# ETM-Code/eirgrid

Hardware: AMD Instinct MI355X
Metric: 26-year episodes/sec (higher is better)
Workload: dtype f64

## Files before the change

eirgrid_amd/csrc/eg_api.cpp:

```cpp
#include <algorithm>
#include <cstdlib>
#include <cstring>

#include "eg_device_tables.h"
#include "eg_host.h"
#include "eg_policy_internal.h"

namespace eg {
namespace {
thread_local std::string g_error;
}
void set_error(const std::string& s) { g_error = s; }
}

using namespace eg;

void eg_host_tables::index() {
  auto F = [&](const char* n, const std::vector<double>& v) { f64[n] = {v.data(), (int64_t)v.size()}; };
  auto I = [&](const char* n, const std::vector<int32_t>& v) { i32[n] = {v.data(), (int64_t)v.size()}; };
  F("usage", H.usage); F("population", H.population); F("pre_co2", H.pre_co2); F("pre_tg", H.pre_tg); F("pre_ig", H.pre_ig);
  F("pre_sg", H.pre_sg); F("pre_optot", H.pre_optot); F("te", H.te); F("coastf", H.coastf); F("dr", H.dr); F("m03", H.m03);
  F("t12", H.t12); F("cc", H.cc); F("out_mw", H.out_mw); F("co2_t", H.co2_t); F("offv", H.offv); F("offc", H.offc);
  F("inflation", H.inflation); F("carbon_price", H.carbon_price);
  f64["size_factor"] = {&H.size_factor, 1};
// ... 4 lines not shown
namespace {
struct Options {
  bool helper_off = false, helper_all = false;
  bool heavy_slots_auto = true; uint32_t heavy_slots_wanted = 4096;
  uint32_t heavy_slots_max = 0;
  bool side_stream_plain = false;
  bool replay_hoist = false;
  int coop_force = 0;
  bool solo_on = true;
  uint32_t solo_tiles = 1u;
};
Options read_options() {
  Options o;
  if (const char* hv = std::getenv("EIRGRID_HELPER_WAVES")) { o.helper_off = std::string(hv) == "0"; o.helper_all = std::string(hv) == "all"; }
  if (const char* hs = std::getenv("EIRGRID_HEAVY_SLOTS")) { o.heavy_slots_wanted = (uint32_t)std::strtoul(hs, nullptr, 10); o.heavy_slots_auto = false; }
  o.heavy_slots_max = uint32_t((size_t(64) << 30) / (size_t(kRadiusClasses) * 2624 * sizeof(double)));
  if (const char* hg = std::getenv("EIRGRID_HEAVY_POOL_GB"))
    o.heavy_slots_max = uint32_t(std::min(double((1u << 20) - 1u), std::max(0.0, std::atof(hg)) * double(size_t(1) << 30) / double(size_t(kRadiusClasses) * 2624 * sizeof(double))));
  if (o.heavy_slots_max > (1u << 20) - 1u) o.heavy_slots_max = (1u << 20) - 1u;
  if (o.heavy_slots_wanted > o.heavy_slots_max) o.heavy_slots_wanted = o.heavy_slots_max;
  if (const char* sp = std::getenv("EIRGRID_SIDE_STREAM")) o.side_stream_plain = std::string(sp) == "plain";
  if (const char* rh = std::getenv("EIRGRID_REPLAY_HOIST")) o.replay_hoist = rh[0] == '1';
  if (const char* cf = std::getenv("EIRGRID_COOP_FORCE")) o.coop_force = std::atoi(cf);
  if (const char* so = std::getenv("EIRGRID_REPLAY_SOLO")) o.solo_on = so[0] != '0';
  if (const char* st = std::getenv("EIRGRID_SOLO_TILES")) o.solo_tiles = st[0] != '0' ? 1u : 0u;
  return o;
}

int collect_timing(eg_ctx* c, int count = -1) {
  if (count < 0 || count > c->ring_pending) count = c->ring_pending;
  for (; count > 0; --count) {
    const int i = (c->ring_head - c->ring_pending + 2 * eg_ctx::kTimingRing) % eg_ctx::kTimingRing;
    const bool heavy = c->ev_used[i] & 1, lean = c->ev_used[i] & 2;
    float best = 0.f, sum = 0.f;
    for (int a = 0; a < 2; ++a)
      for (int b = 0; b < 2; ++b) {
        if (!(a ? lean : heavy) || !(b ? lean : heavy)) continue;
        EG_HIP(hipEventSynchronize(c->ev[i][2 * b + 1]));
        float ms = 0.f;
        EG_HIP(hipEventElapsedTime(&ms, c->ev[i][2 * a], c->ev[i][2 * b + 1]));
        if (a == b) sum += ms;
        if (ms > best) best = ms;
      }
    c->total_ms += double(best); c->grids_ms += double(sum); c->n_launches += 1; c->ring_pending -= 1;
  }
  return EG_OK;
}
}
static bool env_starts(const char* name, char ch) { const char* e = std::getenv(name); return e && e[0] == ch; }
bool eg::stats_replicas_off() { static const bool off = env_starts("EIRGRID_STATS_REPLICAS", '0'); return off; }
bool eg::fetch_full() { static const bool full = env_starts("EIRGRID_FETCH_FULL", '1'); return full; }

int eg::ensure_outputs(eg_ctx* c, uint32_t n) {
  const size_t bytes = size_t(n) * rec::stride + size_t(n) * sizeof(double);
  if (bytes <= c->d_out.count) return EG_OK;
  c->out = DevOut{};
  EG_HIP(c->d_out.reserve(bytes));
  c->out.base = c->d_out;
  c->out.score_list = reinterpret_cast<double*>(c->out.base + size_t(n) * rec::stride);
  EG_HIP(hipMemset(c->out.base, 0, bytes));
  return EG_OK;
}

int eg::ring_take(eg_ctx* c, RolloutPlan& plan, int& slot) {
  if (c->ring_pending == eg_ctx::kTimingRing) EG_TRY(collect_timing(c, 1));
  slot = c->ring_head;
  for (int k = 0; k < 4; ++k) plan.ev[k] = c->ev[slot][k];
  return EG_OK;
}
void eg::ring_commit(eg_ctx* c, int slot, int ev_used) {
  c->ev_used[slot] = uint8_t(ev_used);
  c->ring_head = (c->ring_head + 1) % eg_ctx::kTimingRing; c->ring_pending += 1;
}
int eg::arm_solo(eg_ctx* c, RolloutPlan& plan, uint32_t n) {
  if (!c->solo_on) return EG_OK;
  bool fresh = false;
  EG_HIP(c->d_solo.reserve(n, &fresh));
  if (fresh) EG_HIP(hipMemsetAsync(c->d_solo, 0, sizeof(unsigned long long) * n, nullptr));
  plan.solo_seq = ++c->solo_seq; plan.d_solo = c->d_solo;
  return EG_OK;
}

int eg::prepare_heavy(eg_ctx* c, uint32_t n_heavy, bool known_short) {
  constexpr size_t kSlotBytes = size_t(kRadiusClasses) * 2624 * sizeof(double), kTileBytes = size_t(kMaxVariants) * 64 * sizeof(double);
  if (known_short && !c->dev.heavy) n_heavy = 0;
  uint32_t want = c->heavy_slots_wanted;
  if (c->heavy_slots_auto && want > 0) {
    while (want < n_heavy && want < c->heavy_slots_max) want = want * 2u < c->heavy_slots_max ? want * 2u : c->heavy_slots_max;
  }
  if (want > 0 && n_heavy > 0 && (!c->dev.heavy || want > c->dev.heavy_slots)) {
    if (c->dev.heavy) {
      EG_HIP(hipDeviceSynchronize());
      c->d_heavy.release();
      c->dev.heavy = nullptr; c->dev.heavy_slots = 0; c->dev.heavy_tiles = nullptr;
    }
    if (!c->dev.heavy_claim) {
      if (!c->d_heavy_claim.try_reserve(16)) { c->heavy_slots_wanted = 0; want = 0; }
      else { EG_HIP(hipMemset(c->d_heavy_claim, 0xFF, 64)); c->dev.heavy_claim = c->d_heavy_claim; }
    }
    while (want > 0 && !c->d_heavy.try_reserve((kSlotBytes + kTileBytes) * want)) {
      want = want > 4096u ? want / 2u : 0u;
      c->heavy_slots_auto = false; c->heavy_slots_wanted = want;
    }
    if (want > 0) {
      c->dev.heavy = c->d_heavy; c->dev.heavy_slots = want;
      c->dev.heavy_tiles = reinterpret_cast<double*>(c->d_heavy + kSlotBytes * want);
    }
  }
  c->launch_epoch = (c->launch_epoch + 1u) & 0xFFFu;
  if (c->launch_epoch == 0xFFFu) c->launch_epoch = 0u;
  c->dev.heavy_epoch = c->launch_epoch;
  return EG_OK;
}

namespace {
int launch_batch(eg_ctx* c, uint64_t seed, uint64_t first_index, uint32_t n, const uint8_t* host_mask, uint32_t period, long long* d_stats) {
  if (n == 0) return EG_OK;
  RolloutPlan plan{};
  plan.helper_waves = n <= c->helper_max_episodes;
  plan.n_lean = n;
  const uint8_t* d_mask = nullptr;
  if (host_mask) {
    EG_HIP(c->d_mask.reserve(n));
    EG_HIP(c->d_index.reserve(n));
    std::vector<uint32_t> idx(n);
    uint32_t nh = 0;
    for (uint32_t i = 0; i < n; ++i) if (host_mask[i]) idx[nh++] = i;
    uint32_t k = nh;
    for (uint32_t i = 0; i < n; ++i) if (!host_mask[i]) idx[k++] = i;
    EG_HIP(hipMemcpy(c->d_mask, host_mask, n, hipMemcpyHostToDevice));
    EG_HIP(hipMemcpy(c->d_index, idx.data(), sizeof(uint32_t) * n, hipMemcpyHostToDevice));
    d_mask = c->d_mask;
    plan.n_heavy = nh; plan.n_lean = n - nh; plan.mode = 1u; plan.d_index = c->d_index;
  } else if (period == 1u) {
    plan.n_heavy = n; plan.n_lean = 0;
  } else if (period > 1u) {
    plan.off = uint32_t((uint64_t(period) - first_index % period) % period);
    plan.n_heavy = plan.off < n ? (n - plan.off + period - 1u) / period : 0u;
    plan.n_lean = n - plan.n_heavy; plan.mode = 2u; plan.period = period;
  }
  int slot = 0;
  EG_TRY(ring_take(c, plan, slot));
  const bool split = plan.n_heavy > 0 && plan.n_lean > 0;
  plan.stream_heavy = split ? c->stream_heavy : nullptr;
  plan.stream_lean = nullptr;
  bool list_long = c->long_list_hint;
  if (!c->list_exact && c->h_list_len) list_long = *(volatile uint32_t*)c->h_list_len > uint32_t(kShortReplayMax);
  plan.skip_long = c->list_exact && !list_long;
  EG_TRY(prepare_heavy(c, plan.n_heavy, plan.skip_long));
  if (d_stats != nullptr) {
    const bool off = stats_replicas_off();
    if (!off && n >= 4096u) {
      bool fresh = false;
      EG_HIP(c->d_stats_rep.reserve(size_t(kStatsReplicas) * EG_STATS_LEN, &fresh));
      if (fresh) EG_HIP(hipMemsetAsync(c->d_stats_rep, 0, sizeof(long long) * size_t(kStatsReplicas) * EG_STATS_LEN, nullptr));
    }
    plan.d_stats_rep = (off || n < 4096u) ? nullptr : c->d_stats_rep;
    if (plan.d_stats_rep != nullptr && c->stats_rep_dirty) {
      if (c->stream_heavy) EG_HIP(hipStreamSynchronize(c->stream_heavy));
      EG_HIP(hipMemsetAsync(c->d_stats_rep, 0, sizeof(long long) * size_t(kStatsReplicas) * EG_STATS_LEN, nullptr));
      c->stats_rep_dirty = false;
    }
  }
  if (plan.n_heavy > 0 && !plan.helper_waves && !plan.skip_long && !c->hoist_on)
    EG_TRY(arm_solo(c, plan, plan.n_heavy));
  if (c->hoist_on && plan.n_heavy > 0) {
    plan.hoist_seq = ++c->hoist_seq; plan.d_hoist = reinterpret_cast<HoistInfo*>(c->d_hoist.ptr); plan.coop_out = c->d_coop; plan.coop_force = c->coop_force;
    c->hoist_batches += 1;
  }
  if (split) {
    EG_HIP(hipEventRecord(c->ev_fork[slot], nullptr));
    EG_HIP(hipStreamWaitEvent(c->stream_heavy, c->ev_fork[slot], 0));
    if (list_long || plan.hoist_seq != 0ull) plan.go_event = c->ev_go[slot];
  }
  if (plan.d_stats_rep != nullptr) c->stats_rep_dirty = true;
  EG_LAUNCH("k_rollout", launch_rollout(c->dev, c->snap, c->out, seed, first_index, n, d_mask, period, d_stats, plan));
  if (split) {
    EG_HIP(hipEventRecord(c->ev_join[slot], c->stream_heavy));
    EG_HIP(hipStreamWaitEvent(nullptr, c->ev_join[slot], 0));
  }
  if (d_stats != nullptr && plan.d_stats_rep != nullptr) {
    EG_LAUNCH("k_fold_stats", launch_fold_stats(plan.d_stats_rep, d_stats, nullptr));
    c->stats_rep_dirty = false;
  }
  if (c->fold_mode != 0) EG_TRY(best_result_fold(c, n, first_index));
  if (c->topk_mode != 0) EG_TRY(topk_fold(c, n, first_index, d_stats != nullptr && c->topk_mode == 1));
  if (c->pareto_cap != 0) EG_TRY(pareto_fold(c, n, first_index));
  ring_commit(c, slot, (plan.n_heavy > 0 ? 1 : 0) | (plan.n_lean > 0 ? 2 : 0));
  c->last_n = n; c->last_first = first_index;
  return EG_OK;
// ... 373 lines not shown
```

eirgrid_amd/csrc/eg_internal.h:

```cpp
#pragma once
#include <cstddef>
#include <cstdint>
#include <string>
#include <vector>

#include "eirgrid_hip.h"

namespace eg {

constexpr int kYears = EG_YEARS;
constexpr int kTypes = EG_N_TYPES;
constexpr int kCells = EG_CELLS;
constexpr int kGrid = EG_GRID;
constexpr int kRadiusClasses = 6;
constexpr int kMaxReach = 12;
constexpr int kMults = 3;
constexpr int kOffsetTypes = 4;
constexpr int kPsStride = 2624;
constexpr int kDrCompact = 352;
constexpr int kLdsGens = EG_ONCHIP_GENS;
constexpr int kShortReplayMax = 96;
constexpr int kMaxVariants = 12;
constexpr int kTileW = 8;
constexpr int kTileCols = (kGrid + kTileW - 1) / kTileW;
// ... 8 lines not shown
  std::vector<int32_t> pre_opcnt;
  std::vector<double> te;
  std::vector<double> coastf;
  std::vector<double> dr;
  double size_factor;
  std::vector<double> m03;
  std::vector<double> t12;
  std::vector<double> cc;
  std::vector<double> out_mw;
  std::vector<double> co2_t;
  std::vector<int32_t> cls;
  std::vector<int32_t> rclass;
  std::vector<int32_t> marine;
  std::vector<int32_t> reach;
  std::vector<double> offv;
  std::vector<double> offc;
  std::vector<double> inflation;
  std::vector<double> carbon_price;
  std::vector<int32_t> existing_online;
};

void build_tables(const eg_world& w, HostTables& t);

#ifdef __HIPCC__
#define EG_HD __host__ __device__
#else
#define EG_HD
#endif

struct PsRec { double te, cf, m03; uint32_t cell, pad; };
static_assert(sizeof(PsRec) == 32, "candidate record");

namespace tab {
constexpr size_t a16(size_t x) { return (x + 15) & ~size_t(15); }
constexpr size_t usage = 0;
constexpr size_t population = usage + 8 * kYears;
constexpr size_t pre_co2 = population + 8 * kYears;
constexpr size_t pre_tg = pre_co2 + 8 * kYears;
constexpr size_t pre_ig = pre_tg + 8 * kYears;
constexpr size_t pre_sg = pre_ig + 8 * kYears;
constexpr size_t pre_optot = pre_sg + 8 * kYears;
constexpr size_t inflation = pre_optot + 8 * kYears;
constexpr size_t carbon_price = inflation + 8 * kYears;
constexpr size_t out_mw = carbon_price + 8 * kYears;
constexpr size_t co2_t = out_mw + 8 * 16;
constexpr size_t pre_opcnt = co2_t + 8 * 16;
constexpr size_t variant = a16(pre_opcnt + 4 * kYears);
constexpr size_t cls = variant + 4 * 16;
constexpr size_t rclass = cls + 4 * 16;
constexpr size_t marine = rclass + 4 * 16;
constexpr size_t reach = marine + 4 * 16;
constexpr size_t dr = a16(reach + 4 * 8);
constexpr size_t m03 = a16(dr + 8 * kRadiusClasses * 169);
constexpr size_t t12 = a16(m03 + 8 * kCells);
constexpr size_t offv = a16(t12 + 8 * kYears * kTypes);
constexpr size_t offc = a16(offv + 8 * kYears * kOffsetTypes * kYears);
constexpr size_t cc = a16(offc + 8 * kYears * kOffsetTypes * kMults);
constexpr size_t ps = a16(cc + 8 * size_t(kYears) * kTypes * kYears * kMults * 2);
constexpr size_t hv_box = a16(ps + sizeof(PsRec) * size_t(kYears) * kMaxVariants * kPsStride);
constexpr size_t dr_meta = a16(hv_box + 4 * (1024 + 16));
constexpr size_t dr_compact = a16(dr_meta + 4 * 16);
constexpr size_t pbase = a16(dr_compact + 8 * size_t(kDrCompact));
constexpr size_t pcell = a16(pbase + 8 * size_t(kYears) * kMaxVariants * kPcStride);
constexpr size_t hv_lists = a16(pcell + 4 * size_t(kYears) * kMaxVariants * kPcStride);
constexpr size_t hv_quads = a16(hv_lists + 4 * size_t(64) * 1024);
constexpr size_t te_cell = a16(hv_quads + 4 * 64);
constexpr size_t coastf = a16(te_cell + 8 * size_t(kYears) * kRadiusClasses * kCells);
constexpr size_t cbase = a16(coastf + 8 * size_t(kCells));
constexpr size_t crank = a16(cbase + 8 * size_t(kYears) * kMaxVariants * kCells);
constexpr size_t ucell = a16(crank + 2 * size_t(kYears) * kMaxVariants * kCells);
constexpr size_t umax = a16(ucell + 8 * size_t(kMaxVariants) * kCells);
constexpr size_t rmax = a16(umax + 8 * size_t(kMaxVariants) * 64);
constexpr size_t total = a16(rmax + 8 * size_t(kYears) * kMaxVariants * 64);
}

struct DevTables {
  const uint8_t* base;
  double size_factor;
  int32_t n_existing;
  int32_t n_variants;
  uint32_t heavy_slots, heavy_epoch;
  uint8_t* heavy;
  unsigned* heavy_claim;
  double* heavy_tiles;
  uint32_t solo_tiles;
#define EG_TAB(name, type) EG_HD const type* name() const { return reinterpret_cast<const type*>(base + tab::name); }
  EG_TAB(usage, double) EG_TAB(population, double)
  EG_TAB(pre_co2, double) EG_TAB(pre_tg, double) EG_TAB(pre_ig, double) EG_TAB(pre_sg, double) EG_TAB(pre_optot, double)
  EG_TAB(inflation, double) EG_TAB(carbon_price, double) EG_TAB(out_mw, double) EG_TAB(co2_t, double)
  EG_TAB(pre_opcnt, int32_t) EG_TAB(variant, int32_t) EG_TAB(cls, int32_t) EG_TAB(rclass, int32_t) EG_TAB(marine, int32_t)
  EG_TAB(reach, int32_t)
  EG_TAB(dr, double) EG_TAB(m03, double) EG_TAB(t12, double) EG_TAB(offv, double) EG_TAB(offc, double) EG_TAB(cc, double)
  EG_TAB(ps, PsRec) EG_TAB(pbase, double) EG_TAB(pcell, uint32_t) EG_TAB(hv_lists, uint32_t) EG_TAB(hv_quads, int32_t) EG_TAB(dr_meta, int32_t) EG_TAB(dr_compact, double)
  EG_TAB(te_cell, double) EG_TAB(coastf, double) EG_TAB(cbase, double) EG_TAB(crank, uint16_t) EG_TAB(ucell, double) EG_TAB(umax, double) EG_TAB(rmax, double)
#undef EG_TAB
};

struct DevState {
  double learning_rate, exploration_rate;
  double best_metrics[4];
  double rel_improvement, immediate_weight;
  double p_best_score, p_threshold, p_adaptive_lr, p_stagnation;
  double boost_others, boost_noop, eps_main, scaled_power;
  uint32_t stall, iteration_count;
  int32_t has_best, has_cw, noop_boost, has_lists, p_forced;
  uint32_t heur_min, heur_max;
  uint32_t n_improvements;
  int32_t improved_last;
  uint32_t failed_total;
};
static_assert(sizeof(DevState) % 8 == 0, "state layout");
struct DevImprovement { double score, metrics[4]; uint32_t iteration, pad; };

namespace snap {
constexpr size_t kBestCap = 4096;
constexpr int kPolRow = 128, kPolTotMain = 61, kPolTotDeficit = 62, kPolTotCount = 63, kPolDw = 64, kPolScaledTotal = 79, kPolCw = 80;
constexpr int kPolYear = 101;
constexpr size_t pol = 0;
constexpr size_t scaled = pol + 8 * EG_YEARS * kPolRow;
constexpr size_t scaled_perm = scaled + 8 * EG_YEARS * 64;
constexpr size_t best_mask = scaled_perm + 64 * EG_YEARS;
constexpr size_t bestd_mask = best_mask + 8 * EG_YEARS;
constexpr size_t best_off = bestd_mask + 8 * EG_YEARS;
constexpr size_t bestd_off = best_off + 4 * 28;
constexpr size_t best_actions = bestd_off + 4 * 28;
constexpr size_t bestd_actions = best_actions + kBestCap;
constexpr size_t state = (bestd_actions + kBestCap + 15) & ~size_t(15);
constexpr size_t kPlanStride = state - best_mask;
static_assert(kPlanStride == 8832 && kPlanStride % 64 == 0, "plan block layout");
constexpr size_t upload_bytes = state + sizeof(DevState);
constexpr int kImpLogCap = 256;
constexpr size_t best_w = (upload_bytes + 15) & ~size_t(15);
constexpr size_t imp_log = best_w + 8 * EG_YEARS * EG_N_ACTIONS;
constexpr size_t best_rec_state = (imp_log + sizeof(DevImprovement) * kImpLogCap + 63) & ~size_t(63);
constexpr size_t best_rec = best_rec_state + 64;
}

struct DevSnapshot {
  const uint8_t* base;
  int32_t enable_energy_sales;
  int32_t write_yearly;
  double learning_rate, exploration_rate;
  uint32_t stall;
  int32_t has_best;
  int32_t has_cw;
  int32_t noop_boost;
  double rel_improvement;
  double immediate_weight;
  int32_t has_best_actions, has_best_deficit;
  uint32_t heur_min, heur_max;
  double boost_others, boost_noop;
  double eps_main;
  double scaled_power;
  const uint8_t* lists;
  const uint8_t* plan_pool;
#define EG_SNAP(name, type) EG_HD const type* name() const { return reinterpret_cast<const type*>(base + snap::name); }
#define EG_LIST(name, type) EG_HD const type* name() const { return reinterpret_cast<const type*>(lists + (snap::name - snap::best_mask)); }
  EG_SNAP(pol, double) EG_SNAP(scaled, double) EG_SNAP(scaled_perm, uint8_t)
  EG_LIST(best_mask, unsigned long long) EG_LIST(bestd_mask, unsigned long long)
  EG_LIST(best_off, int32_t) EG_LIST(bestd_off, int32_t) EG_LIST(best_actions, uint8_t) EG_LIST(bestd_actions, uint8_t)
  EG_SNAP(state, DevState)
#undef EG_LIST
#undef EG_SNAP
  EG_HD int32_t resident_list_len() const { return reinterpret_cast<const int32_t*>(base + snap::best_off)[EG_YEARS]; }
};

namespace rec {
// ... 194 lines not shown
```

eirgrid_amd/csrc/eg_replay_solo.h:

```cpp
#pragma once

namespace solo {

struct Lists {
  unsigned long long gen_pack;
  __device__ __forceinline__ static int* words() { return reinterpret_cast<int*>(sm.pol); }
  __device__ __forceinline__ int gpack_at(int i) const {
    __builtin_amdgcn_fence(__ATOMIC_RELEASE, "workgroup");
    return tail_u16(gen_pack, i);
  }
  __device__ __forceinline__ void gpack_put(int, int) const {}
  __device__ __forceinline__ void opack_put(int, int) const {}
  __device__ __forceinline__ int cls(int t) const { return (sm.type_info[t] >> 12) & 3; }
  __device__ __forceinline__ double out(int t) const { return sm.type_out[t]; }
  __device__ __forceinline__ void year_end(int yi, int ngen, int noff) const { words()[yi] = ngen; words()[EG_YEARS + yi] = noff; }
  __device__ __forceinline__ void finish(int run_pos, int def_pos, int act_pos, int ngen, int noff, unsigned long long bytes) const {
    int* w = words();
    w[52] = run_pos; w[53] = def_pos; w[54] = act_pos; w[55] = ngen; w[56] = noff;
    *reinterpret_cast<unsigned long long*>(w + 58) = bytes;
  }
};
static_assert(snap::kPolRow * 8 >= 60 * 4, "the script's lengths fit the policy row block");

constexpr int kEnt = 8;
struct Entries { int base[kEnt], delta[kEnt], dd[kEnt]; double fac[kEnt]; };
__device__ __forceinline__ void load_entries(Entries& E, int lane) {
#pragma unroll
  for (int k = 0; k < kEnt; ++k) {
    const uint32_t en = sh2.box[k * kWave + lane];
    const int rc = (int)(en >> 19), di = (int)(en & 31u) - 16, dj = (int)((en >> 5) & 31u) - 16;
    E.base[k] = rc * kFieldStride; E.delta[k] = di * kGrid + dj; E.dd[k] = (di & 0xFFFF) | (int)((unsigned)dj << 16);
    E.fac[k] = factor_by_q<false>(rc, (int)offsetof(Smem, dr), (int)((en >> 10) & 511u));
  }
}
template <int kN>
__device__ __forceinline__ void field_add(unsigned long long field_addr, const Entries& E, int cell) {
  const GlobalF64 base = (GlobalF64)field_addr;
  const int gi = cell / kGrid, gj = cell - gi * kGrid;
  double val[kN]; int off[kN];
#pragma unroll
  for (int k = 0; k < kN; ++k) {
    const int ci = gi + (int)(short)(E.dd[k] & 0xFFFF), cj = gj + (E.dd[k] >> 16);
    const bool inside = (unsigned)ci < (unsigned)kGrid && (unsigned)cj < (unsigned)kGrid;
    off[k] = E.base[k] + (inside ? cell + E.delta[k] : kCells);
    val[k] = field_load(base + off[k]);
  }
#pragma unroll
  for (int k = 0; k < kN; ++k) base[off[k]] = val[k] * E.fac[k];
}

}

__global__ void __launch_bounds__(kWave, EG_HEAVY_WAVES) k_replay_solo(DevTables T, DevSnapshot S_in, DevOut O, unsigned long long first_index, uint32_t n_episodes,
                                                                       const uint8_t* __restrict__ replay_mask, uint32_t replay_period, long long* stats,
                                                                       EpisodeMap emap) {
  const int lane = threadIdx.x;
  if (blockIdx.x >= emap.count) return;
  if (S_in.plan_pool == nullptr && !(S_in.state()->has_lists && S_in.resident_list_len() > kShortReplayMax)) return;
  if (emap.hoist_seq != 0ull && *emap.hoist == emap.hoist_seq) return;
  const uint32_t e = map_episode(emap, blockIdx.x);
  if (e >= n_episodes) return;
  DevSnapshot S = S_in;
  load_state(S);
  plan_lists(S, e);
  const bool replay = replay_mask != nullptr ? replay_mask[e] != 0 : (replay_period != 0u && S.has_best_actions && (first_index + e) % replay_period == 0ull);
  if (!replay || !S.has_best_actions) return;
#ifdef EG_SOLO_STAMPS
  unsigned long long cs[8] = {0, 0, 0, 0, 0, 0, 0, 0}, cs_last = __builtin_readcyclecounter();
#define EG_SS(slot) do { const unsigned long long now_ = __builtin_readcyclecounter(); cs[slot] += now_ - cs_last; cs_last = now_; } while (0)
#else
#define EG_SS(slot) do {} while (0)
#endif
  load_static_tables(T, lane, true);
#if defined(EG_SOLO_STAMPS) && defined(EG_STAMPS)
  if (lane < 8) sm.hdbg[lane >> 2][lane & 3] = 0ull;
#endif
  wave_sync();
  EG_SS(0);

  solo::Lists ls{(unsigned long long)O.gen_pack(e)};
  if (!rs::script(T, S, O, e, ls, lane)) return;
  __builtin_amdgcn_fence(__ATOMIC_RELEASE, "workgroup");
  wave_sync();
  EG_SS(1);
  const int* words = solo::Lists::words();
  const int n_gens = __builtin_amdgcn_readfirstlane(words[55]);

  Episode ep;
  ep.ngen = 0; ep.chunks = 0; ep.heavy = -1; ep.heavy_classes = 0; ep.heavy_quads = 0;
  uint16_t* gen_cell = O.gen_cell(e);
  const ListTail tail = {(unsigned long long)gen_cell, (unsigned long long)O.gen_pack(e), (unsigned long long)O.off_pack(e)};
  PrefixCache prefix_cache0 = {0.0, -1, 0};
  uint32_t search_seq = 0;
  int tile_variants = 0;
  int pk_block = 0;
  solo::Entries E;
#pragma unroll
  for (int k = 0; k < solo::kEnt; ++k) { E.base[k] = 0; E.delta[k] = 0; E.dd[k] = 0; E.fac[k] = 1.0; }
  for (int g = 0; g < n_gens; ++g) {
    if ((g & (kWave - 1)) == 0) pk_block = g + lane < n_gens ? tail_u16(tail.gen_pack, g + lane) : 0;
    const int pk = __builtin_amdgcn_readlane(pk_block, g & (kWave - 1));
    const int t = pk & 15, yi = (pk >> 4) & 31, m = pk >> 9;
    double m03v = 0.0;
    int cell = -1;
    bool placed = false;
    auto between = [] {};
    EG_SS(2);
    if (ep.ngen >= kHeavyGens && ep.heavy != -2) {
      const unsigned long long slot_bytes = (unsigned long long)(kRadiusClasses * kFieldStride) * 8ull;
      if (ep.heavy == -1) ep.heavy = heavy_claim(T, lane);
      if (ep.heavy >= 0) {
        const int info = __builtin_amdgcn_readfirstlane(sm.type_info[t]);
        const int hv = info & 15, hrc = (info >> 4) & 15;
        const unsigned long long class_addr = (unsigned long long)T.heavy + (unsigned long long)ep.heavy * slot_bytes + (unsigned long long)(hrc * kFieldStride) * 8ull;
        const unsigned long long tiles_addr = (unsigned long long)T.heavy_tiles + (unsigned long long)((ep.heavy * kMaxVariants + hv) * 64) * 8ull;
        if (!((ep.heavy_classes >> hrc) & 1)) {
          heavy_build_class<false>(class_addr, tail.gen_cell, lane, hrc, throughput_table(info), (info >> 8) & 15, ep.ngen);
          ep.heavy_classes |= 1 << hrc;
          ep.heavy_quads = __builtin_amdgcn_readfirstlane(T.hv_quads()[ep.heavy_classes]);
          wave_sync();
#pragma unroll
          for (int k = 0; k < kBoxLds / kWave; ++k) sh2.box[k * kWave + lane] = T.hv_lists()[ep.heavy_classes * 1024 + k * kWave + lane];
          wave_sync();
          solo::load_entries(E, lane);
        }
        int hr = kTilesUndecided;
        if (T.solo_tiles && !((tile_variants >> hv) & 1)) {
          ((GlobalF64)tiles_addr)[lane] = T.umax()[hv * 64 + lane];
          tile_variants |= 1 << hv;
        }
        if (T.solo_tiles) hr = place_tiles((unsigned long long)T.base, yi * kMaxVariants + hv, class_addr, tiles_addr, tail.gen_cell, T.size_factor, lane, hrc, throughput_table(info), ep.ngen);
        if (hr == kTilesUndecided) {
          const size_t yv = (size_t)(yi * kMaxVariants + hv) * kPsStride, yc = (size_t)(yi * kMaxVariants + hv) * kPcStride;
          hr = place_heavy<false>((unsigned long long)(T.ps() + yv), (unsigned long long)(T.pbase() + yc), (unsigned long long)(T.pcell() + yc), class_addr,
                                  tail.gen_cell, T.size_factor, lane, hrc, throughput_table(info), ep.ngen);
        }
        if (hr >= 0) { cell = hr & 0xFFFF; ep.chunks += hr >> 16; placed = true; }
      }
    }
    if (!placed && ep.ngen > kLdsGens) {
      const int info = __builtin_amdgcn_readfirstlane(sm.type_info[t]);
      const int xr = place_exact_long<false>((unsigned long long)(T.ps() + (size_t)(yi * kMaxVariants + (info & 15)) * kPsStride), tail.gen_cell,
                                             T.size_factor, lane, (info >> 4) & 15, throughput_table(info), ep.ngen);
      cell = xr < 0 ? -1 : (xr & 0xFFFF);
      if (xr >= 0) ep.chunks += xr >> 16;
      placed = true;
    }
    if (!placed) cell = __builtin_amdgcn_readfirstlane(place_search<0>(T, lane, yi, t, ep.ngen, nullptr, &m03v, prefix_cache0, between, ep.chunks, &search_seq));
    EG_SS(3);
    if (cell >= 0 && ep.heavy_classes != 0) {
      const unsigned long long field_addr = (unsigned long long)T.heavy + (unsigned long long)ep.heavy * ((unsigned long long)(kRadiusClasses * kFieldStride) * 8ull);
      ep.chunks += 2 * ep.heavy_quads;
      const unsigned long long hv_list = (unsigned long long)(T.hv_lists() + ep.heavy_classes * 1024);
      if (ep.heavy_quads == 1) solo::field_add<4>(field_addr, E, cell);
      else solo::field_add<8>(field_addr, E, cell);
      if (ep.heavy_quads == 3) heavy_add_body<false, 4>(field_addr, hv_list, lane, cell, 8);
      else if (ep.heavy_quads >= 4) heavy_add_body<false, 8>(field_addr, hv_list, lane, cell, 8);
    }
    if (cell < 0) {
      if (lane == 0 && ep.heavy >= 0) emap.solo[blockIdx.x] = (emap.solo_seq << 21) | (1ull << 20) | (unsigned long long)ep.heavy;
      return;
    }
    if (lane == 0) {
      if (ep.ngen < kLdsGens) { sm.gcell[ep.ngen] = (uint16_t)(cell | (t << 12)); sm.gbm[ep.ngen] = (uint8_t)(yi | (m << 5)); }
      gen_cell[ep.ngen] = (uint16_t)cell;
    }
    wave_sync();
    ep.ngen += 1;
    EG_SS(4);
  }

  __builtin_amdgcn_fence(__ATOMIC_RELEASE, "workgroup");
  wave_sync();
  double total_cost = 0.0, total_credit = 0.0, total_sales = 0.0;
  double last[7] = {0.0, 0.0, 0.0, 0.0, 0.0, 0.0, 0.0};
  for (int y0 = 0; y0 < kYears; y0 += 4) {
    const rs::YearRow q = rs::books_quad(T, S_in, O, e, y0, words, words + EG_YEARS, lane, [](const uint16_t* list, int i) { return tail_u16((unsigned long long)list, i); });
#pragma unroll
    for (int r = 0; r < 4; ++r) {
      const int yi = y0 + r;
      if (yi >= kYears) break;
#pragma unroll
      for (int k = 0; k < 7; ++k) last[k] = readlane_f64(q.v[k], 16 * r);
      total_cost = yi == 0 ? last[0] : total_cost + last[0];
      total_credit = yi == 0 ? last[1] : total_credit + last[1];
      total_sales = yi == 0 ? last[2] : total_sales + last[2];
      if (S_in.write_yearly && lane == 0) {
        double* row = O.yearly(e) + yi * EG_YEARLY_FIELDS;
        row[EG_Y_TOTAL_COST] = total_cost; row[EG_Y_TOTAL_CREDIT] = total_credit; row[EG_Y_TOTAL_SALES] = total_sales;
      }
    }
  }
  EG_SS(5);
  if (lane == 0) {
    O.metrics(e)[0] = last[3]; O.metrics(e)[1] = last[4]; O.metrics(e)[2] = last[5];
    O.metrics(e)[3] = last[6] >= 0.0 ? 1.0 : 0.0;
    *O.status(e) = EG_EP_OK; *O.n_gens(e) = words[55]; *O.n_offsets(e) = words[56];
    *O.n_draws(e) = 0ull;
    *O.bytes_moved(e) = (double)*reinterpret_cast<const unsigned long long*>(words + 58);
    *O.n_chunks(e) = (uint32_t)ep.chunks;
  }
  if (stats != nullptr) {
    __builtin_amdgcn_fence(__ATOMIC_RELEASE, "workgroup");
    __builtin_amdgcn_fence(__ATOMIC_ACQUIRE, "workgroup");
    wave_sync();
    StatsParams P;
    load_stats_params(S, P);
    episode_update_stats(O, S, P, e, lane, stats, 1ull, emap.stats_rep ? (int)(blockIdx.x % (uint32_t)kStatsReplicas) : -1);
  }
  EG_SS(6);
#ifdef EG_SOLO_STAMPS
  if (lane == 0) {
    unsigned long long* dbg = (unsigned long long*)(O.act_log(e) + EG_ACT_CAP - 256);
    for (int i = 0; i < 8; ++i) dbg[i] = cs[i];
// ... 9 lines not shown
```

eirgrid_amd/csrc/eg_rollout.hip:

```cpp
#include <hip/hip_runtime.h>
#include <cstddef>
#include <hip/hip_ext.h>

#include "eg_internal.h"

#define EG_DETPOW_QUAL __device__ __forceinline__
#include "eg_detpow.h"
#define EG_RM __device__ __forceinline__
#include "eg_reduced_math.h"

namespace eg {
namespace {

constexpr int kWave = 64;
constexpr int kD2Max = 144, kD2Stride = 146;
constexpr int kCmdYear = 1 << 30;
constexpr int kHelperWaves = 1;
constexpr int kSpinCap = 1 << 20;
constexpr int kSearchLost = -2;
constexpr double kMinWeight = 0.0001;
constexpr double kMaxWeight = 0.999;
constexpr double kMaxCost = 50000000000.0;
constexpr int kBattery = 12, kPeaker = 8;
constexpr int kNothing = 60, kFirstOffset = 45, kFirstOther = 57;
// ... 981 lines not shown
__device__ __noinline__ int place_heavy(unsigned long long list_addr, unsigned long long pb_addr, unsigned long long pc_addr, unsigned long long class_addr,
                                        unsigned long long tail_cells, double size_factor, int lane, int rc, int tbl, int ngen) {
#ifdef EG_STAMPS
  const unsigned long long ts0 = __builtin_readcyclecounter();
#endif
  asm volatile("s_waitcnt vmcnt(0)" ::: "memory");
  const int ngen_s = __builtin_amdgcn_readfirstlane(ngen);
  constexpr int kChunks = (kCells + kWave - 1) / kWave;
  constexpr int kGroup = 4, kGroups = (kChunks + kGroup - 1) / kGroup;
  constexpr double kKeep = 1.0 - 0x1p-30;
  double M = 0.0; int K = 0;
  double lm = 0.0, l2 = 0.0; int lcell = 0;
  auto uniform_u64 = [](unsigned long long a) { return ((unsigned long long)(unsigned)__builtin_amdgcn_readfirstlane((int)(a >> 32)) << 32) | (unsigned)__builtin_amdgcn_readfirstlane((int)a); };
  const unsigned long long pb_s = uniform_u64(pb_addr), pc_s = uniform_u64(pc_addr), a_s = uniform_u64(class_addr);
  auto pb_at = [&](int r) { return *(GlobalF64c)(pb_s + (unsigned long long)((unsigned)r * 8u)); };
  auto pc_at = [&](int r) { return *(GlobalI32c)(pc_s + (unsigned long long)((unsigned)r * 4u)); };
  auto field_at = [&](int cell) { return __hip_atomic_load((GlobalF64)(a_s + (unsigned long long)((unsigned)cell * 8u)), __ATOMIC_RELAXED, __HIP_MEMORY_SCOPE_AGENT); };
  static_assert((kGroups + 1) * kGroup * kWave <= kPcStride, "the scan requests a round ahead");
  double cb[kGroup], nb[kGroup]; int cc[kGroup], nc[kGroup];
#pragma unroll
  for (int j = 0; j < kGroup; ++j) { cb[j] = pb_at(j * kWave + lane); cc[j] = pc_at(j * kWave + lane); }
#define EG_SCAN_ROUND(CB, CC, NB, NC, g_)                                                                                        \
  {                                                                                                                              \
    if ((g_) >= kGroups || ((g_) > 0 && !(readlane_f64(CB[0], 0) >= M * kKeep))) break;       \
    double ap[kGroup];                                                                                                           \
    _Pragma("unroll") for (int j = 0; j < kGroup; ++j) ap[j] = field_at(CC[j]);                                                  \
    _Pragma("unroll") for (int j = 0; j < kGroup; ++j) { NB[j] = pb_at((((g_) + 1) * kGroup + j) * kWave + lane); NC[j] = pc_at((((g_) + 1) * kGroup + j) * kWave + lane); } \
    _Pragma("unroll") for (int j = 0; j < kGroup; ++j) {                                                                         \
      const double v = CB[j] * ap[j];                                                                                            \
      const double key = __hiloint2double(__double2hiint(v), (__double2loint(v) & ~63) | ((g_) * kGroup + j));                   \
      const bool larger = key > lm;                                                                                              \
      l2 = vmax64(l2, vmin64(lm, key));                                                      \
      lm = vmax64(lm, key);                                                                                                      \
      lcell = larger ? CC[j] : lcell;                                                                                            \
    }                                                                                                                            \
    M = __hiloint2double((int)wave_max_u32((unsigned)__double2hiint(lm)), 0);       \
    K = ((g_) + 1) * kGroup < kChunks ? ((g_) + 1) * kGroup : kChunks;                                                           \
  }
#pragma nounroll
  for (int g = 0;; g += 2) {
    EG_SCAN_ROUND(cb, cc, nb, nc, g)
    EG_SCAN_ROUND(nb, nc, cb, cc, g + 1)
  }
#undef EG_SCAN_ROUND
  M = wave_max_f64(lm);
  if (!(M >= 1e-250)) return kSearchFallback;
#ifdef EG_STAMPS
  const unsigned long long ts1 = __builtin_readcyclecounter();
#endif
  const double thr = M * kKeep;
  int ncand = 0, solo = -1;
  if (__ballot(l2 >= thr) == 0ull) {
    const unsigned long long m1 = __ballot(lm >= thr);
    ncand = __popcll(m1);
    if (ncand == 1) solo = __ffsll((long long)m1) - 1;
    if ((m1 >> lane) & 1ull) sm.gstage[1][__popcll(m1 & ((1ull << lane) - 1ull))] = (__double2loint(lm) & 63) * kWave + lane;
  } else {
    for (int k = 0; k < K; ++k) {
      const double approx = pb_at(k * kWave + lane) * field_at(pc_at(k * kWave + lane));
      const unsigned long long m = __ballot(approx >= thr && approx > 0.0);
      if (m != 0ull) {
        const int pos = ncand + __popcll(m & ((1ull << lane) - 1ull));
        if (((m >> lane) & 1ull) && pos < kWave) sm.gstage[1][pos] = k * kWave + lane;
        ncand += __popcll(m);
      }
    }
  }
  if (ncand > kWave || ncand == 0) return kSearchFallback;
  wave_sync();
#ifdef EG_STAMPS
  asm volatile("s_waitcnt vmcnt(0)" ::: "memory");
  const unsigned long long ts2 = __builtin_readcyclecounter();
#endif
  const ChunkBest b = heavy_exact<kLatency>(list_addr, tail_cells, size_factor, lane, rc, tbl, ngen_s, ncand, ncand == 1 && solo >= 0 ? __builtin_amdgcn_readlane(lcell, solo) : -1);
  if (!(b.score > 0.0)) return kSearchFallback;
#ifdef EG_STAMPS
  if (lane == 0) { sm.hdbg[0][0] += ts1 - ts0; sm.hdbg[0][1] += ts2 - ts1; sm.hdbg[0][2] += __builtin_readcyclecounter() - ts2; sm.hdbg[1][0] += (unsigned long long)K; sm.hdbg[1][1] += (unsigned long long)ncand; sm.hdbg[1][2] += 1ull; }
#endif
  return heavy_result(b, lane, K, ncand);
}

constexpr int kTilesUndecided = -4;
static_assert(kTileW * kTileW == kWave, "a cell of a tile per lane");
__device__ __noinline__ int place_tiles(unsigned long long tab_addr, int yv, unsigned long long class_addr, unsigned long long tiles_addr,
                                        unsigned long long tail_cells, double size_factor, int lane, int rc, int tbl, int ngen) {
#ifdef EG_STAMPS
  const unsigned long long ts0 = __builtin_readcyclecounter();
#endif
  asm volatile("s_waitcnt vmcnt(0)" ::: "memory");
  const int ngen_s = __builtin_amdgcn_readfirstlane(ngen);
  constexpr int kChunks = (kCells + kWave - 1) / kWave, kGroup = 4, kGroups = (kChunks + kGroup - 1) / kGroup;
  constexpr double kKeep = 1.0 - 0x1p-30, kKeepTile = 1.0 - 0x1p-29;
  constexpr int kNoTile = 63;
  static_assert(kNoTile >= kTiles && (kNoTile / kTileCols) * kTileW >= kGrid, "kNoTile is off the grid");
  auto uniform_u64 = [](unsigned long long a) { return ((unsigned long long)(unsigned)__builtin_amdgcn_readfirstlane((int)(a >> 32)) << 32) | (unsigned)__builtin_amdgcn_readfirstlane((int)a); };
  const unsigned long long tab_s = uniform_u64(tab_addr), a_s = uniform_u64(class_addr), t_s = uniform_u64(tiles_addr);
  const unsigned long long yv_s = (unsigned long long)(unsigned)__builtin_amdgcn_readfirstlane(yv);
  const unsigned long long cb_s = tab_s + tab::cbase + yv_s * (8ull * kCells), rk_s = tab_s + tab::crank + yv_s * (2ull * kCells);
  const unsigned long long pb_s = tab_s + tab::pbase + yv_s * (8ull * kPcStride), rm_s = tab_s + tab::rmax + yv_s * (8ull * 64);
  const unsigned long long uc_s = tab_s + tab::ucell + (yv_s % kMaxVariants) * (8ull * kCells);
  const GlobalF64 gmax = (GlobalF64)t_s;
  auto field_at = [&](int cell) { return __hip_atomic_load((GlobalF64)(a_s + (unsigned long long)((unsigned)cell * 8u)), __ATOMIC_RELAXED, __HIP_MEMORY_SCOPE_AGENT); };
  auto cb_at = [&](int cell) { return *(GlobalF64c)(cb_s + (unsigned long long)((unsigned)cell * 8u)); };
  auto uc_at = [&](int cell) { return *(GlobalF64c)(uc_s + (unsigned long long)((unsigned)cell * 8u)); };
  auto rk_at = [&](int cell) { return (int)*(const uint16_t __attribute__((address_space(1)))*)(rk_s + (unsigned long long)((unsigned)cell * 2u)); };
  const double gb = lane >= 1 && lane < kGroups ? *(GlobalF64c)(pb_s + (unsigned long long)((unsigned)(lane * kGroup * kWave) * 8u)) : 0.0;
  const double bound = lane < kTiles ? *(GlobalF64c)(rm_s + (unsigned long long)((unsigned)lane * 8u)) * field_load(gmax + lane) : 0.0;
  unsigned long long left = __ballot(bound > 0.0);
  if (left == 0ull) return kSearchFallback;
  const unsigned hb = (unsigned)__double2hiint(bound);
  const unsigned h1 = wave_max_u32(hb);
  int ta = __ffsll((long long)(left & __ballot(hb == h1))) - 1, tb = kNoTile;
  {
    const unsigned long long rest = left & ~(1ull << ta);
    const unsigned h2 = wave_max_u32(lane == ta ? 0u : hb);
    const unsigned long long second = rest & __ballot(hb == h2);
    if (rest != 0ull) tb = __ffsll((long long)(second != 0ull ? second : rest)) - 1;
  }
  double lm = 0.0, l2 = 0.0;
  int lrank = 0, lcell = -1;
#ifdef EG_STAMPS
  int tiles = 0;
#endif
  auto fold = [&](double v, int r, int c) {
    const double key = __hiloint2double(__double2hiint(v), (__double2loint(v) & ~63) | (r >> 6));
    const bool larger = key > lm;
    l2 = vmax64(l2, vmin64(lm, key));
    lm = vmax64(lm, key);
    lrank = larger ? r : lrank; lcell = larger ? c : lcell;
  };
#pragma nounroll
  for (;;) {
    left &= ~(1ull << ta) & ~(1ull << tb);
    const int ia = (ta / kTileCols) * kTileW + (lane >> 3), ja = (ta % kTileCols) * kTileW + (lane & 7);
    const int ib = (tb / kTileCols) * kTileW + (lane >> 3), jb = (tb % kTileCols) * kTileW + (lane & 7);
    const bool ina = ia < kGrid && ja < kGrid, inb = ib < kGrid && jb < kGrid;
    const int ca = ina ? ia * kGrid + ja : 0, cb = inb ? ib * kGrid + jb : 0;
    const double fa = field_at(ca), fb = field_at(cb), pa = cb_at(ca), pb = cb_at(cb), ua = uc_at(ca), ub = uc_at(cb);
    const int ra = rk_at(ca), rb = rk_at(cb);
    fold(ina ? pa * fa : 0.0, ra, ca);
    fold(inb ? pb * fb : 0.0, rb, cb);
    const unsigned gha = wave_max_u32(ina ? (unsigned)__double2hiint(ua * fa) : 0u), ghb = wave_max_u32(inb ? (unsigned)__double2hiint(ub * fb) : 0u);
    if (lane == 0) {
      gmax[ta] = __hiloint2double((int)gha, -1);
      if (tb < kTiles) gmax[tb] = __hiloint2double((int)ghb, -1);
    }
#ifdef EG_STAMPS
    tiles += tb < kTiles ? 2 : 1;
#endif
    const double m_lo = __hiloint2double((int)wave_max_u32((unsigned)__double2hiint(lm)), 0);
    left &= __ballot(bound >= m_lo * kKeepTile);
    if (left == 0ull) break;
    ta = __ffsll((long long)left) - 1;
    const unsigned long long rest = left & (left - 1ull);
    tb = rest != 0ull ? __ffsll((long long)rest) - 1 : kNoTile;
  }
  const double M = wave_max_f64(lm);
  if (!(M >= 1e-250)) return kSearchFallback;
#ifdef EG_STAMPS
  const unsigned long long ts1 = __builtin_readcyclecounter();
#endif
  const double thr = M * kKeep;
  if (__ballot(l2 >= thr) != 0ull) return kTilesUndecided;
  const int gstar = (__double2loint(M) & 63) / kGroup;
  const double m_hi = __hiloint2double(__double2hiint(M), 0);
  const unsigned long long stops = __ballot(lane > gstar && lane < kGroups && !(gb >= m_hi * kKeep));
  const int g_stop = stops != 0ull ? __ffsll((long long)stops) - 1 : kGroups;
  const int K = kGroup * g_stop < kChunks ? kGroup * g_stop : kChunks;
  const unsigned long long m1 = __ballot(lm >= thr && lrank < K * kWave);
  const int ncand = __popcll(m1);
  if (ncand == 0) return kTilesUndecided;
  if (ncand > 1) {
    unsigned long long seen = 0ull;
    for (unsigned long long m = m1; m != 0ull; m &= m - 1ull) {
      const unsigned long long bit = 1ull << (__builtin_amdgcn_readlane(lrank, __ffsll((long long)m) - 1) & 63);
      if (seen & bit) return kTilesUndecided;
      seen |= bit;
    }
  }
  if ((m1 >> lane) & 1ull) sm.gstage[1][__popcll(m1 & ((1ull << lane) - 1ull))] = lrank;
  wave_sync();
#ifdef EG_STAMPS
  asm volatile("s_waitcnt vmcnt(0)" ::: "memory");
  const unsigned long long ts2 = __builtin_readcyclecounter();
#endif
  const unsigned long long list_addr = tab_s + tab::ps + yv_s * (sizeof(PsRec) * (unsigned long long)kPsStride);
  const ChunkBest b = heavy_exact<false>(list_addr, tail_cells, size_factor, lane, rc, tbl, ngen_s, ncand, ncand == 1 ? __builtin_amdgcn_readlane(lcell, __ffsll((long long)m1) - 1) : -1);
  if (!(b.score > 0.0)) return kSearchFallback;
#ifdef EG_STAMPS
  if (lane == 0) {
    sm.hdbg[0][0] += ts1 - ts0; sm.hdbg[0][1] += ts2 - ts1; sm.hdbg[0][2] += __builtin_readcyclecounter() - ts2;
    sm.hdbg[1][0] += (unsigned long long)K; sm.hdbg[1][1] += (unsigned long long)ncand; sm.hdbg[1][2] += 1ull; sm.hdbg[1][3] += (unsigned long long)tiles;
  }
#endif
  return heavy_result(b, lane, K, ncand);
}

template <bool kLatency>
__device__ __noinline__ int place_exact_long(unsigned long long list_addr, unsigned long long tail_cells, double size_factor, int lane, int rc, int tbl, int ngen) {
  const int ngen_s = __builtin_amdgcn_readfirstlane(ngen);
  const int cap = factor_cap<kLatency>(tbl);
  constexpr int kChunks = (kCells + kWave - 1) / kWave;
  double best = 0.0, m03w = 0.0; int best_c = kCells, chunks = 0;
  for (int chunk = 0; chunk < kChunks; ++chunk) {
    const int r = chunk * kWave + lane;
    const PsRec c = load_rec(list_addr, r);
    const double base = (c.te * c.cf) * size_factor;
    if (chunk > 0 && !(readlane_f64(base, 0) >= best)) break;
    ++chunks;
    const int ci = (int)c.cell / kGrid, cj = (int)c.cell - ci * kGrid;
    double s = c.te;
    for (int gb = 0; gb < ngen_s; gb += kWave) {
      const int mine = list_cell(tail_cells, gb, lane, ngen_s, 0);
      const int cnt = ngen_s - gb < kWave ? ngen_s - gb : kWave;
      for (int j = 0; j < cnt; ++j) {
        const int gc = __builtin_amdgcn_readlane(mine, j);
        const int gi = gc / kGrid, gj = gc - gi * kGrid;
        int q = (ci - gi) * (ci - gi) + (cj - gj) * (cj - gj);
        q = q < cap ? q : cap;
        s = s * factor_by_q<kLatency>(rc, tbl, q);
      }
    }
    s = (s * c.cf) * size_factor;
    s = r < kCells ? s : 0.0;
    if (__any(s > best || (s == best && s > 0.0 && (int)c.cell < best_c))) {
      const ChunkBest b = chunk_reduce<false>(s, (int)c.cell, c.m03);
      if (b.score > best || (b.score == best && b.cell < best_c)) { best = b.score; best_c = b.cell; m03w = b.m03; }
    }
// ... 1588 lines not shown
```

Baseline: 8.695 million.

## Keep per-tile bounds in shared memory instead of the heavy global buffer

Moves the per-variant tile upper bounds used by the solo tile search from a global heavy_tiles buffer into packed 32-bit high words stored in reused LDS regions (opack, pol/rng tail, scaled). The rmax and pbase loads are also hoisted out of place_tiles into the caller and passed in as arguments. This removes global round-trips and device allocation for the tile bounds and shrinks the heavy buffer. The cost is aliasing LDS regions that other code uses, which depends on those regions not being live during the search.

```diff
diff --git a/eirgrid_amd/csrc/eg_api.cpp b/eirgrid_amd/csrc/eg_api.cpp
--- a/eirgrid_amd/csrc/eg_api.cpp
+++ b/eirgrid_amd/csrc/eg_api.cpp
@@ -110,7 +110,7 @@
 }
 
 int eg::prepare_heavy(eg_ctx* c, uint32_t n_heavy, bool known_short) {
-  constexpr size_t kSlotBytes = size_t(kRadiusClasses) * 2624 * sizeof(double), kTileBytes = size_t(kMaxVariants) * 64 * sizeof(double);
+  constexpr size_t kSlotBytes = size_t(kRadiusClasses) * 2624 * sizeof(double);
   if (known_short && !c->dev.heavy) n_heavy = 0;
   uint32_t want = c->heavy_slots_wanted;
   if (c->heavy_slots_auto && want > 0) {
@@ -120,20 +120,17 @@
     if (c->dev.heavy) {
       EG_HIP(hipDeviceSynchronize());
       c->d_heavy.release();
-      c->dev.heavy = nullptr; c->dev.heavy_slots = 0; c->dev.heavy_tiles = nullptr;
+      c->dev.heavy = nullptr; c->dev.heavy_slots = 0;
     }
     if (!c->dev.heavy_claim) {
       if (!c->d_heavy_claim.try_reserve(16)) { c->heavy_slots_wanted = 0; want = 0; }
       else { EG_HIP(hipMemset(c->d_heavy_claim, 0xFF, 64)); c->dev.heavy_claim = c->d_heavy_claim; }
     }
-    while (want > 0 && !c->d_heavy.try_reserve((kSlotBytes + kTileBytes) * want)) {
+    while (want > 0 && !c->d_heavy.try_reserve(kSlotBytes * want)) {
       want = want > 4096u ? want / 2u : 0u;
       c->heavy_slots_auto = false; c->heavy_slots_wanted = want;
     }
-    if (want > 0) {
-      c->dev.heavy = c->d_heavy; c->dev.heavy_slots = want;
-      c->dev.heavy_tiles = reinterpret_cast<double*>(c->d_heavy + kSlotBytes * want);
-    }
+    if (want > 0) { c->dev.heavy = c->d_heavy; c->dev.heavy_slots = want; }
   }
   c->launch_epoch = (c->launch_epoch + 1u) & 0xFFFu;
   if (c->launch_epoch == 0xFFFu) c->launch_epoch = 0u;
diff --git a/eirgrid_amd/csrc/eg_internal.h b/eirgrid_amd/csrc/eg_internal.h
--- a/eirgrid_amd/csrc/eg_internal.h
+++ b/eirgrid_amd/csrc/eg_internal.h
@@ -114,7 +114,6 @@
   uint32_t heavy_slots, heavy_epoch;
   uint8_t* heavy;
   unsigned* heavy_claim;
-  double* heavy_tiles;
   uint32_t solo_tiles;
 #define EG_TAB(name, type) EG_HD const type* name() const { return reinterpret_cast<const type*>(base + tab::name); }
   EG_TAB(usage, double) EG_TAB(population, double)
diff --git a/eirgrid_amd/csrc/eg_replay_solo.h b/eirgrid_amd/csrc/eg_replay_solo.h
--- a/eirgrid_amd/csrc/eg_replay_solo.h
+++ b/eirgrid_amd/csrc/eg_replay_solo.h
@@ -21,6 +21,18 @@
   }
 };
 static_assert(snap::kPolRow * 8 >= 60 * 4, "the script's lengths fit the policy row block");
+
+constexpr int kBoundWords = kTiles, kBoundsPerBlock = 5, kLengthBytes = 60 * 4;
+__device__ __forceinline__ int tile_bounds(int hv) {
+  static_assert(kBoundsPerBlock * kBoundWords * 4 <= (int)sizeof(Smem::opack), "five variants' bounds in sm.opack");
+  static_assert(offsetof(Smem, rng) == offsetof(Smem, pol) + sizeof(Smem::pol), "sm.rng follows sm.pol");
+  static_assert(kLengthBytes + kBoundsPerBlock * kBoundWords * 4 <= (int)(sizeof(Smem::pol) + sizeof(Smem::rng)), "five behind the script's lengths, up to the end of sm.rng");
+  static_assert((kMaxVariants - 2 * kBoundsPerBlock) * kBoundWords * 4 <= (int)sizeof(Smem::scaled) && kMaxVariants >= 2 * kBoundsPerBlock, "the rest in sm.scaled");
+  static_assert(offsetof(Smem, opack) % 4 == 0 && offsetof(Smem, pol) % 4 == 0 && offsetof(Smem, scaled) % 4 == 0, "words");
+  const int block = hv / kBoundsPerBlock;
+  const int base = block == 0 ? (int)offsetof(Smem, opack) : block == 1 ? (int)offsetof(Smem, pol) + kLengthBytes : (int)offsetof(Smem, scaled);
+  return base + (hv - block * kBoundsPerBlock) * (kBoundWords * 4);
+}
 
 constexpr int kEnt = 8;
 struct Entries { int base[kEnt], delta[kEnt], dd[kEnt]; double fac[kEnt]; };
@@ -113,7 +125,7 @@
         const int info = __builtin_amdgcn_readfirstlane(sm.type_info[t]);
         const int hv = info & 15, hrc = (info >> 4) & 15;
         const unsigned long long class_addr = (unsigned long long)T.heavy + (unsigned long long)ep.heavy * slot_bytes + (unsigned long long)(hrc * kFieldStride) * 8ull;
-        const unsigned long long tiles_addr = (unsigned long long)T.heavy_tiles + (unsigned long long)((ep.heavy * kMaxVariants + hv) * 64) * 8ull;
+        const int tiles_off = solo::tile_bounds(hv);
         if (!((ep.heavy_classes >> hrc) & 1)) {
           heavy_build_class<false>(class_addr, tail.gen_cell, lane, hrc, throughput_table(info), (info >> 8) & 15, ep.ngen);
           ep.heavy_classes |= 1 << hrc;
@@ -126,10 +138,21 @@
         }
         int hr = kTilesUndecided;
         if (T.solo_tiles && !((tile_variants >> hv) & 1)) {
-          ((GlobalF64)tiles_addr)[lane] = T.umax()[hv * 64 + lane];
+          if (lane < solo::kBoundWords) reinterpret_cast<uint32_t*>(reinterpret_cast<char*>(&sm) + tiles_off)[lane] = (uint32_t)__double2hiint(T.umax()[hv * 64 + lane]);
           tile_variants |= 1 << hv;
         }
-        if (T.solo_tiles) hr = place_tiles((unsigned long long)T.base, yi * kMaxVariants + hv, class_addr, tiles_addr, tail.gen_cell, T.size_factor, lane, hrc, throughput_table(info), ep.ngen);
+        if (T.solo_tiles) {
+          constexpr int kGroups = ((kCells + kWave - 1) / kWave + 3) / 4;
+          static_assert(kGroups * 4 * kWave <= kPcStride && kGroups <= kWave, "the boundaries are entries of the list, a lane each");
+          const int yv = yi * kMaxVariants + hv;
+          static_assert(tab::total < (1ull << 32), "32-bit offsets into the tables");
+          const unsigned long long tab_base = (unsigned long long)T.base;
+          int lane_here = lane;
+          asm volatile("" : "+v"(lane_here));
+          const double rmax_l = *(GlobalF64c)(tab_base + (unsigned long long)((unsigned)tab::rmax + (unsigned)(yv * 64 + lane) * 8u));
+          const double gb_l = *(GlobalF64c)(tab_base + (unsigned long long)((unsigned)tab::pbase + (unsigned)(yv * kPcStride + (lane_here < kGroups ? lane_here : kGroups - 1) * (4 * kWave)) * 8u));
+          hr = place_tiles((unsigned long long)T.base, yv, class_addr, tiles_off, rmax_l, gb_l, tail.gen_cell, T.size_factor, lane, hrc, throughput_table(info), ep.ngen);
+        }
         if (hr == kTilesUndecided) {
           const size_t yv = (size_t)(yi * kMaxVariants + hv) * kPsStride, yc = (size_t)(yi * kMaxVariants + hv) * kPcStride;
           hr = place_heavy<false>((unsigned long long)(T.ps() + yv), (unsigned long long)(T.pbase() + yc), (unsigned long long)(T.pcell() + yc), class_addr,
diff --git a/eirgrid_amd/csrc/eg_rollout.hip b/eirgrid_amd/csrc/eg_rollout.hip
--- a/eirgrid_amd/csrc/eg_rollout.hip
+++ b/eirgrid_amd/csrc/eg_rollout.hip
@@ -1087,7 +1087,7 @@
 
 constexpr int kTilesUndecided = -4;
 static_assert(kTileW * kTileW == kWave, "a cell of a tile per lane");
-__device__ __noinline__ int place_tiles(unsigned long long tab_addr, int yv, unsigned long long class_addr, unsigned long long tiles_addr,
+__device__ __noinline__ int place_tiles(unsigned long long tab_addr, int yv, unsigned long long class_addr, int tiles_off, double rmax_l, double gb,
                                         unsigned long long tail_cells, double size_factor, int lane, int rc, int tbl, int ngen) {
 #ifdef EG_STAMPS
   const unsigned long long ts0 = __builtin_readcyclecounter();
@@ -1099,18 +1099,16 @@
   constexpr int kNoTile = 63;
   static_assert(kNoTile >= kTiles && (kNoTile / kTileCols) * kTileW >= kGrid, "kNoTile is off the grid");
   auto uniform_u64 = [](unsigned long long a) { return ((unsigned long long)(unsigned)__builtin_amdgcn_readfirstlane((int)(a >> 32)) << 32) | (unsigned)__builtin_amdgcn_readfirstlane((int)a); };
-  const unsigned long long tab_s = uniform_u64(tab_addr), a_s = uniform_u64(class_addr), t_s = uniform_u64(tiles_addr);
+  const unsigned long long tab_s = uniform_u64(tab_addr), a_s = uniform_u64(class_addr);
   const unsigned long long yv_s = (unsigned long long)(unsigned)__builtin_amdgcn_readfirstlane(yv);
   const unsigned long long cb_s = tab_s + tab::cbase + yv_s * (8ull * kCells), rk_s = tab_s + tab::crank + yv_s * (2ull * kCells);
-  const unsigned long long pb_s = tab_s + tab::pbase + yv_s * (8ull * kPcStride), rm_s = tab_s + tab::rmax + yv_s * (8ull * 64);
   const unsigned long long uc_s = tab_s + tab::ucell + (yv_s % kMaxVariants) * (8ull * kCells);
-  const GlobalF64 gmax = (GlobalF64)t_s;
+  uint32_t* const gmax = reinterpret_cast<uint32_t*>(reinterpret_cast<char*>(&sm) + __builtin_amdgcn_readfirstlane(tiles_off));
   auto field_at = [&](int cell) { return __hip_atomic_load((GlobalF64)(a_s + (unsigned long long)((unsigned)cell * 8u)), __ATOMIC_RELAXED, __HIP_MEMORY_SCOPE_AGENT); };
   auto cb_at = [&](int cell) { return *(GlobalF64c)(cb_s + (unsigned long long)((unsigned)cell * 8u)); };
   auto uc_at = [&](int cell) { return *(GlobalF64c)(uc_s + (unsigned long long)((unsigned)cell * 8u)); };
   auto rk_at = [&](int cell) { return (int)*(const uint16_t __attribute__((address_space(1)))*)(rk_s + (unsigned long long)((unsigned)cell * 2u)); };
-  const double gb = lane >= 1 && lane < kGroups ? *(GlobalF64c)(pb_s + (unsigned long long)((unsigned)(lane * kGroup * kWave) * 8u)) : 0.0;
-  const double bound = lane < kTiles ? *(GlobalF64c)(rm_s + (unsigned long long)((unsigned)lane * 8u)) * field_load(gmax + lane) : 0.0;
+  const double bound = lane < kTiles ? rmax_l * __hiloint2double((int)gmax[lane], -1) : 0.0;
   unsigned long long left = __ballot(bound > 0.0);
   if (left == 0ull) return kSearchFallback;
   const unsigned hb = (unsigned)__double2hiint(bound);
@@ -1147,8 +1145,8 @@
     fold(inb ? pb * fb : 0.0, rb, cb);
     const unsigned gha = wave_max_u32(ina ? (unsigned)__double2hiint(ua * fa) : 0u), ghb = wave_max_u32(inb ? (unsigned)__double2hiint(ub * fb) : 0u);
     if (lane == 0) {
-      gmax[ta] = __hiloint2double((int)gha, -1);
-      if (tb < kTiles) gmax[tb] = __hiloint2double((int)ghb, -1);
+      gmax[ta] = gha;
+      if (tb < kTiles) gmax[tb] = ghb;
     }
 #ifdef EG_STAMPS
     tiles += tb < kTiles ? 2 : 1;
```

Measured after the change: 8.725 million, median of 6. About the same (+0.4%).
